# mrlooi/PoseCNN

Hardware: AMD Instinct MI355X
Metric: frames/sec 640x480x21-class Hough-vote+RoI+ADD-loss, 1/2/4/8 MI355X (higher is better)
Workload: dtype f32 (FC GEMMs: exact 3-way split-bf16 x6 MFMA, products within 2^-24, fp32 accumulate: fp32-faithful)

## Files before the change

include/posecnn_hip.h:

```cpp
#ifndef POSECNN_HIP_H
#define POSECNN_HIP_H

#include <stddef.h>
#include <stdint.h>

#ifdef __cplusplus
extern "C" {
#endif

#define PCNN_OK 0
#define PCNN_EINVAL 1
#define PCNN_EHIP 2
#define PCNN_ECAPACITY 3

#define PCNN_MAX_ROI 128

int pcnn_abi_version(void);
const char* pcnn_strerror(int code);

int pcnn_set_completion_event(void* event);
int pcnn_completion_event_pending(void);

size_t pcnn_hough_voting_workspace_size(int B, int H, int W, int C, int skip_pixels, float vote_thr);

// ... 35 lines not shown
int pcnn_roi_pool_fwd_pair(const float* data_a, int Ha, int Wa, float scale_a, const float* data_b, int Hb, int Wb,
                           float scale_b, int B, int C, const float* rois, int R_cap, int roi_stride,
                           int batch_base, const int32_t* num_rois_dev, int pooled_h, int pooled_w, float* top_sum,
                           int32_t* argmax_a, int32_t* argmax_b, void* stream);

int pcnn_roi_pool_fwd_pair_px(const float* data_a, int Ha, int Wa, float scale_a, const float* data_b, int Hb,
                              int Wb, float scale_b, int B, int C, const float* rois, int R_cap, int roi_stride,
                              int batch_base, const int32_t* num_rois_dev, int pooled_h, int pooled_w,
                              float* top_sum, uint16_t* argmax_a, uint16_t* argmax_b, void* stream);

size_t pcnn_roi_pool_bwd_workspace_size(int B, int R_cap);

int pcnn_roi_pool_bwd(const float* top_diff, const int32_t* argmax, int B, int H, int W, int C, int layout,
                      const float* rois, int R_cap, int roi_stride, int batch_base, const int32_t* num_rois_dev,
                      float spatial_scale, int pooled_h, int pooled_w, int pool_channel, float* bottom_diff,
                      void* workspace, size_t workspace_bytes, void* stream);

int pcnn_roi_pool_bwd_px(const float* top_diff, const uint16_t* argmax_px, int B, int H, int W, int C,
                         const float* rois, int R_cap, int roi_stride, int batch_base, const int32_t* num_rois_dev,
                         float spatial_scale, int pooled_h, int pooled_w, float* bottom_diff, void* workspace,
                         size_t workspace_bytes, void* stream);

size_t pcnn_add_loss_workspace_size(int R_cap, int C, int P);

int pcnn_add_loss_fwd(const float* pred, const float* target, const float* weight, const float* points,
                      const float* symmetry, int R_cap, const int32_t* num_rois_dev, int C, int P, float margin,
                      int loss_norm_rows, const int32_t* loss_norm_rows_dev, float* loss, float* bottom_diff,
                      void* workspace, size_t workspace_bytes, void* stream);

int pcnn_add_loss_prep(const float* weight, const float* symmetry, int R_cap, const int32_t* num_rois_dev, int C,
                       int P, void* workspace, size_t workspace_bytes, void* stream);
int pcnn_add_loss_fwd_prepared(const float* pred, const float* target, const float* weight, const float* points,
                               const float* symmetry, int R_cap, const int32_t* num_rois_dev, int C, int P,
                               float margin, int loss_norm_rows, const int32_t* loss_norm_rows_dev, float* loss,
                               float* bottom_diff, void* workspace, size_t workspace_bytes, void* stream);

int pcnn_add_loss_fwd_head_bwd(const float* pred, const float* target, const float* weight, const float* points,
                               const float* symmetry, int R_cap, const int32_t* num_rois_dev, int C, int P,
                               float margin, int loss_norm_rows, const int32_t* loss_norm_rows_dev,
                               float* bottom_diff, void* workspace, size_t workspace_bytes, const float* tanh_out,
                               const float* d_pred_scale, float* d_y8, void* stream);
int pcnn_add_loss_total(int R_cap, const int32_t* num_rois_dev, int C, int P, const void* workspace,
                        size_t workspace_bytes, float* loss, void* stream);

int pcnn_add_loss_bwd(const float* top_diff, const float* bottom_diff, int n, const int32_t* num_rois_dev,
                      int row_len, float* out, void* stream);
// ... 145 lines not shown
```

posecnn_amd/_lib.py:

```python
import ctypes
import os
import threading

import torch

_HERE = os.path.dirname(os.path.abspath(__file__))
LIB_PATH = os.environ.get("POSECNN_HIP_LIB") or os.path.join(_HERE, "libposecnn_hip.so")

_lib = None
_lock = threading.Lock()

c_int = ctypes.c_int
c_float = ctypes.c_float
c_size_t = ctypes.c_size_t
c_void_p = ctypes.c_void_p

_SIGS = {
    "pcnn_abi_version": (c_int, []),
    "pcnn_strerror": (ctypes.c_char_p, [c_int]),
    "pcnn_set_completion_event": (c_int, [c_void_p]),
    "pcnn_completion_event_pending": (c_int, []),
    "pcnn_hough_voting_workspace_size": (c_size_t, [c_int, c_int, c_int, c_int, c_int, c_float]),
    "pcnn_hough_voting": (c_int, [c_void_p, c_void_p, c_void_p, c_void_p, c_int, c_void_p, c_int, c_int, c_int,
                                  c_int, c_int, c_int, c_int, c_int, c_float, c_int, c_float, c_float, c_int,
# ... 5 lines not shown
                                       c_int, c_void_p, c_void_p, c_size_t, c_void_p]),
    "pcnn_hough_voting_compact": (c_int, [c_void_p, c_void_p, c_void_p, c_void_p, c_int, c_void_p, c_int, c_int,
                                          c_int, c_int, c_int, c_int, c_int, c_int, c_float, c_int, c_float, c_float,
                                          c_int, c_void_p, c_void_p, c_void_p, c_void_p, c_void_p, c_void_p, c_int,
                                          c_void_p, c_void_p, c_size_t, c_void_p]),
    "pcnn_hough_voting_grad": (c_int, [c_void_p, c_void_p, c_int, c_int, c_int, c_int, c_void_p]),
    "pcnn_hough_voting_diag": (c_int, [c_void_p, c_int, c_int, c_int, c_int, c_int, c_float, c_void_p, c_void_p]),
    "pcnn_roi_pool_fwd": (c_int, [c_void_p, c_int, c_int, c_int, c_int, c_int, c_void_p, c_int, c_int, c_int,
                                  c_void_p, c_float, c_int, c_int, c_int, c_void_p, c_void_p, c_void_p]),
    "pcnn_roi_pool_fwd_accumulate": (c_int, [c_void_p, c_int, c_int, c_int, c_int, c_int, c_void_p, c_int, c_int,
                                             c_int, c_void_p, c_float, c_int, c_int, c_int, c_void_p, c_void_p, c_void_p]),
    "pcnn_roi_pool_fwd_pair": (c_int, [c_void_p, c_int, c_int, c_float, c_void_p, c_int, c_int, c_float, c_int, c_int,
                                       c_void_p, c_int, c_int, c_int, c_void_p, c_int, c_int, c_void_p, c_void_p,
                                       c_void_p, c_void_p]),
    "pcnn_roi_pool_fwd_pair_px": (c_int, [c_void_p, c_int, c_int, c_float, c_void_p, c_int, c_int, c_float, c_int,
                                          c_int, c_void_p, c_int, c_int, c_int, c_void_p, c_int, c_int, c_void_p,
                                          c_void_p, c_void_p, c_void_p]),
    "pcnn_roi_pool_bwd_workspace_size": (c_size_t, [c_int, c_int]),
    "pcnn_roi_pool_bwd_px": (c_int, [c_void_p, c_void_p, c_int, c_int, c_int, c_int, c_void_p, c_int, c_int, c_int,
                                     c_void_p, c_float, c_int, c_int, c_void_p, c_void_p, c_size_t, c_void_p]),
    "pcnn_roi_pool_bwd": (c_int, [c_void_p, c_void_p, c_int, c_int, c_int, c_int, c_int, c_void_p, c_int, c_int,
                                  c_int, c_void_p, c_float, c_int, c_int, c_int, c_void_p, c_void_p, c_size_t, c_void_p]),
    "pcnn_add_loss_workspace_size": (c_size_t, [c_int, c_int, c_int]),
    "pcnn_add_loss_fwd": (c_int, [c_void_p, c_void_p, c_void_p, c_void_p, c_void_p, c_int, c_void_p, c_int, c_int,
                                  c_float, c_int, c_void_p, c_void_p, c_void_p, c_void_p, c_size_t, c_void_p]),
    "pcnn_add_loss_fwd_prepared": (c_int, [c_void_p, c_void_p, c_void_p, c_void_p, c_void_p, c_int, c_void_p, c_int, c_int,
                                  c_float, c_int, c_void_p, c_void_p, c_void_p, c_void_p, c_size_t, c_void_p]),
    "pcnn_add_loss_prep": (c_int, [c_void_p, c_void_p, c_int, c_void_p, c_int, c_int, c_void_p, c_size_t, c_void_p]),
    "pcnn_add_loss_fwd_head_bwd": (c_int, [c_void_p, c_void_p, c_void_p, c_void_p, c_void_p, c_int, c_void_p, c_int,
                                           c_int, c_float, c_int, c_void_p, c_void_p, c_void_p, c_size_t, c_void_p,
                                           c_void_p, c_void_p, c_void_p]),
    "pcnn_add_loss_total": (c_int, [c_int, c_void_p, c_int, c_int, c_void_p, c_size_t, c_void_p, c_void_p]),
    "pcnn_add_loss_bwd": (c_int, [c_void_p, c_void_p, c_int, c_void_p, c_int, c_void_p, c_void_p]),
    "pcnn_div_rn_check": (c_int, [c_void_p, c_float, c_int, c_int, c_void_p, c_void_p]),
    "pcnn_backproject_fwd": (c_int, [c_void_p, c_void_p, c_void_p, c_void_p, c_int, c_void_p, c_int, c_int, c_int,
                                     c_int, c_int, c_int, c_int, c_float, c_void_p, c_void_p, c_void_p, c_void_p]),
    "pcnn_backproject_bwd": (c_int, [c_void_p, c_void_p, c_void_p, c_int, c_int, c_int, c_int, c_int, c_int,
                                     c_void_p, c_void_p]),
    "pcnn_gemm_workspace_size": (c_size_t, [c_int, c_int, c_int, c_int, c_int]),
    "pcnn_gemm": (c_int, [c_int, c_int, c_int, c_void_p, c_void_p, c_int, c_int, c_void_p, c_int, c_int, c_void_p,
                          c_int, c_void_p, c_int, c_void_p, c_int, c_void_p, c_void_p, c_int, c_void_p, c_size_t,
                          c_void_p]),
    "pcnn_gemm_drop": (c_int, [c_int, c_int, c_int, c_void_p, c_void_p, c_int, c_int, c_void_p, c_int, c_int,
                               c_void_p, c_int, c_void_p, c_int, c_void_p, c_int, c_void_p, c_int, c_float, c_void_p,
                               c_void_p, c_int, c_void_p, c_size_t, c_void_p]),
    "pcnn_gemm_drop_gen": (c_int, [c_int, c_int, c_int, c_void_p, c_void_p, c_int, c_int, c_void_p, c_int, c_int,
# ... 141 lines not shown
```

posecnn_amd/average_distance_loss/average_distance_loss_op.py:

```python
import warnings

import torch

from .. import _lib


def workspace_bytes(R, num_classes, num_points):
    return _lib.load().pcnn_add_loss_workspace_size(R, num_classes, num_points)


def average_distance_loss_prep(bottom_weight, bottom_symmetry, num_points, workspace, num_rois=None, points=None):
    if points is not None:
        warnings.warn("average_distance_loss_prep: `points` is ignored (the pruned ADD-S search is removed)",
                      DeprecationWarning, stacklevel=2)
    _lib.require_gpu(bottom_weight, bottom_symmetry, workspace)
    w = bottom_weight.contiguous().float()
    R, PC = w.shape
    rc = _lib.load().pcnn_add_loss_prep(_lib.ptr(w), _lib.ptr(bottom_symmetry.contiguous().float()), R,
                                        _lib.ptr(num_rois), PC // 4, int(num_points), _lib.ptr(workspace),
                                        workspace.numel(), _lib.stream_ptr())
    _lib.check(rc, "average_distance_loss_prep")


def average_distance_loss(bottom_prediction, bottom_target, bottom_weight, bottom_point, bottom_symmetry, margin,
                          name=None, num_rois=None, loss_norm_rows=0, loss_norm_rows_dev=None, out=None,
                          workspace=None, prepared=False):
    _lib.require_gpu(bottom_prediction, bottom_target, bottom_weight, bottom_point, bottom_symmetry)
    if margin < 0:
        raise ValueError(f"Need margin >= 0, got {margin}")
    pred = bottom_prediction.contiguous().float()
    R, PC = pred.shape
# ... 64 lines not shown
```

posecnn_amd/csrc/average_distance.hip:

```cpp
#include "pcnn_common.h"
#include "head_common.h"
#include <cfloat>
#include <type_traits>

namespace {

#ifndef ADD_LANES
#define ADD_LANES 64
#endif
constexpr int kSymLanes = ADD_LANES;
#ifndef ADD_GRID
#define ADD_GRID 1024
#endif
#ifndef ADD_PPL
#define ADD_PPL 4
#endif
constexpr int kPPL = ADD_PPL;
constexpr int kPts = kSymLanes * kPPL;
constexpr int kMaxPointsLds = 8192;

__device__ __forceinline__ int rows_of(const int32_t* dev, int cap) {
  if (!dev) return cap;
  int r = *dev;
  return r < cap ? r : cap;
}
// ... 50 lines not shown
                                                float bn, float rbn, double ln, double rln, float* acc) {
  const float dist = (x1 - x2) * (x1 - x2) + (y1 - y2) * (y1 - y2) + (z1 - z2) * (z1 - z2);
  if (dist < margin) return;
  acc[0] += (float)div_rn((double)(dist - margin), ln, rln);
  const float d0[9] = {2 * s, -2 * w, 2 * v, 2 * w, 2 * s, -2 * u, -2 * v, 2 * u, 2 * s};
  const float d1[9] = {2 * u, 2 * v, 2 * w, 2 * v, -2 * u, -2 * s, 2 * w, 2 * s, -2 * u};
  const float d2[9] = {-2 * v, 2 * u, 2 * s, 2 * u, 2 * v, 2 * w, -2 * s, 2 * w, -2 * v};
  const float d3[9] = {-2 * w, -2 * s, 2 * u, 2 * s, -2 * w, 2 * v, 2 * u, 2 * v, 2 * w};
  const float X[3] = {X0, X1, X2};
  const float df[3] = {x1 - x2, y1 - y2, z1 - z2};
  float e0 = 0.f, e1 = 0.f, e2 = 0.f, e3 = 0.f;
#pragma unroll
  for (int a = 0; a < 3; a++)
#pragma unroll
    for (int b = 0; b < 3; b++) {
      e0 += div_rn(df[a] * X[b] * d0[a * 3 + b], bn, rbn);
      e1 += div_rn(df[a] * X[b] * d1[a * 3 + b], bn, rbn);
      e2 += div_rn(df[a] * X[b] * d2[a * 3 + b], bn, rbn);
      e3 += div_rn(df[a] * X[b] * d3[a * 3 + b], bn, rbn);
    }
  acc[1] += e0; acc[2] += e1; acc[3] += e2; acc[4] += e3;
}

__device__ __forceinline__ void add_plain_row(int n, const float* __restrict__ pred, const float* __restrict__ target,
                                              const float* __restrict__ points, const float* __restrict__ symmetry,
                                              int R, int C, int P, float margin, int norm_rows,
                                              const int32_t* __restrict__ norm_rows_dev, int nchunk,
                                              const int32_t* __restrict__ rcls, float* __restrict__ partial,
                                              float (*red)[5]) {
  const int cls = rcls[n];
  if (cls >= 0 && symmetry[cls] > 0) return;
  float* out = partial + (size_t)n * nchunk * 5;
  for (int i = threadIdx.x; i < nchunk * 5; i += blockDim.x) out[i] = 0.f;
  if (cls < 0) return;
  const int PC = 4 * C;
  const float* tq = target + (size_t)n * PC + 4 * cls;
  const float* pq = pred + (size_t)n * PC + 4 * cls;
  float Rg[9], Rp[9];
  quat2rot(tq[0], tq[1], tq[2], tq[3], Rg);
  const float s = pq[0], u = pq[1], v = pq[2], w = pq[3];
  quat2rot(s, u, v, w, Rp);
  const int Rn = norm_rows_dev ? *norm_rows_dev : (norm_rows > 0 ? norm_rows : R);
  const float bn = (float)(Rn * P), rbn = 1.f / bn;
  const double ln = 2.0 * (double)Rn * (double)P, rln = 1.0 / ln;
  const float* pts = points + (size_t)cls * P * 3;
  float acc[5] = {0.f, 0.f, 0.f, 0.f, 0.f};
  for (int p = threadIdx.x; p < P; p += blockDim.x) {
    const float X0 = pts[p * 3 + 0], X1 = pts[p * 3 + 1], X2 = pts[p * 3 + 2];
    const float x1 = Rp[0] * X0 + Rp[1] * X1 + Rp[2] * X2;
    const float y1 = Rp[3] * X0 + Rp[4] * X1 + Rp[5] * X2;
    const float z1 = Rp[6] * X0 + Rp[7] * X1 + Rp[8] * X2;
    const float x2 = Rg[0] * X0 + Rg[1] * X1 + Rg[2] * X2;
    const float y2 = Rg[3] * X0 + Rg[4] * X1 + Rg[5] * X2;
    const float z2 = Rg[6] * X0 + Rg[7] * X1 + Rg[8] * X2;
    add_point_terms(X0, X1, X2, x1, y1, z1, x2, y2, z2, s, u, v, w, margin, bn, rbn, ln, rln, acc);
  }
#pragma unroll
  for (int q = 0; q < 5; q++) acc[q] = pcnn::wave_sum(acc[q]);
  if (pcnn::lane_id() == 0)
    for (int q = 0; q < 5; q++) red[threadIdx.x >> 6][q] = acc[q];
  __syncthreads();
  if (threadIdx.x < 5) {
    float t = 0.f;
    for (int i = 0; i < (int)(blockDim.x >> 6); i++) t += red[i][threadIdx.x];
    out[threadIdx.x] = t;
  }
}

#ifndef ADD_GROUPS
#define ADD_GROUPS 4
#endif
constexpr int kSymGroups = ADD_GROUPS;
constexpr int kSymThreads = kSymLanes * kSymGroups;
#ifndef ADD_BLK
#define ADD_BLK 8
#endif
constexpr int kBlk = ADD_BLK;

__global__ void __launch_bounds__(kSymThreads) k_add_rows(const float* __restrict__ pred,
                                                           const float* __restrict__ target,
                                                           const float* __restrict__ weight,
                                                           const float* __restrict__ points,
                                                           const float* __restrict__ symmetry, int R_cap,
                                                           const int32_t* __restrict__ num_rois_dev, int C, int P,
                                                           float margin, int norm_rows,
                                                           const int32_t* __restrict__ norm_rows_dev, int nchunk,
                                                           const int32_t* __restrict__ rcls,
                                                           const int32_t* __restrict__ sym_rows,
                                                           const int32_t* __restrict__ nsym,
                                                           int32_t* __restrict__ queue,
                                                           float* __restrict__ partial) {
  extern __shared__ __attribute__((aligned(16))) float4 gpts[];
  __shared__ float mdist[kSymGroups - 1][kPts];
  __shared__ int midx[kSymGroups - 1][kPts];
  __shared__ float red[kSymThreads / 64][5];
  __shared__ int s_imin[kPts];
  const int R = rows_of(num_rois_dev, R_cap);
  const int sym_items = *nsym * nchunk;
  const int items = sym_items + R;
  const int grp = threadIdx.x / kSymLanes, lt = threadIdx.x % kSymLanes;
  const int quarter = ((P + kSymGroups - 1) / kSymGroups + kBlk - 1) / kBlk * kBlk;
  const int c0 = grp * quarter, c1 = min(P, c0 + quarter);
  __shared__ int s_item;
  for (;;) {
  __syncthreads();
  if (threadIdx.x == 0) s_item = atomicAdd(queue, 1);
  __syncthreads();
  const int item = s_item;
  if (item >= items) break;
  if (item >= sym_items) {
    add_plain_row(item - sym_items, pred, target, points, symmetry, R, C, P, margin, norm_rows, norm_rows_dev,
                  nchunk, rcls, partial, red);
    continue;
  }
  const int nfull = P / kPts, nsym_rows = *nsym;
  int n, chunk, slot;
  if (item < nsym_rows * nfull) {
    slot = item / nfull;
    chunk = item % nfull;
  } else {
    slot = item - nsym_rows * nfull;
    chunk = nfull;
  }
  n = sym_rows[slot];
  const int PC = 4 * C;
  const int cls = rcls[n];
  float* out = partial + ((size_t)n * nchunk + chunk) * 5;
  const float* tq = target + (size_t)n * PC + 4 * cls;
  const float* pq = pred + (size_t)n * PC + 4 * cls;
  float Rg[9], Rp[9];
  quat2rot(tq[0], tq[1], tq[2], tq[3], Rg);
  const float s = pq[0], u = pq[1], v = pq[2], w = pq[3];
  quat2rot(s, u, v, w, Rp);
  const float* pts = points + (size_t)cls * P * 3;
  for (int i = threadIdx.x; i < P; i += blockDim.x) {
    const float X0 = pts[i * 3 + 0], X1 = pts[i * 3 + 1], X2 = pts[i * 3 + 2];
    gpts[i] = make_float4(Rg[0] * X0 + Rg[1] * X1 + Rg[2] * X2, Rg[3] * X0 + Rg[4] * X1 + Rg[5] * X2,
                          Rg[6] * X0 + Rg[7] * X1 + Rg[8] * X2, 0.f);
  }
  __syncthreads();
  float qx[kPPL], qy[kPPL], qz[kPPL], Xq[kPPL][3];
  int pq_[kPPL];
#pragma unroll
  for (int k = 0; k < kPPL; k++) {
    const int p = chunk * kPts + k * kSymLanes + lt;
    pq_[k] = p;
    const int pp = p < P ? p : 0;
    Xq[k][0] = pts[pp * 3 + 0]; Xq[k][1] = pts[pp * 3 + 1]; Xq[k][2] = pts[pp * 3 + 2];
    qx[k] = Rp[0] * Xq[k][0] + Rp[1] * Xq[k][1] + Rp[2] * Xq[k][2];
    qy[k] = Rp[3] * Xq[k][0] + Rp[4] * Xq[k][1] + Rp[5] * Xq[k][2];
    qz[k] = Rp[6] * Xq[k][0] + Rp[7] * Xq[k][1] + Rp[8] * Xq[k][2];
  }
  auto dist_to = [&](int k, const float4& c) {
    return (qx[k] - c.x) * (qx[k] - c.x) + (qy[k] - c.y) * (qy[k] - c.y) + (qz[k] - c.z) * (qz[k] - c.z);
  };
  float dmin[kPPL];
  int iblk[kPPL];
#pragma unroll
  for (int k = 0; k < kPPL; k++) { dmin[k] = FLT_MAX; iblk[k] = -1; }
  typedef float f2 __attribute__((ext_vector_type(2)));
  f2 px[kPPL / 2], py[kPPL / 2], pz[kPPL / 2];
#pragma unroll
  for (int h = 0; h < kPPL / 2; h++) {
// ... 15 lines not shown
        for (int j = 0; j < kBlk; j++) {
          const f2 ex = px[h] - c[j].x, ey = py[h] - c[j].y, ez = pz[h] - c[j].z;
          d[j] = ex * ex + ey * ey + ez * ez;
        }
#pragma unroll
        for (int e = 0; e < 2; e++) {
          const int k = 2 * h + e;
          float bm = fminf(d[0][e], d[1][e]);
#pragma unroll
          for (int j = 2; j < kBlk; j += 2) bm = fminf(bm, fminf(d[j][e], d[j + 1][e]));
          if (bm < dmin[k]) { dmin[k] = bm; iblk[k] = i; }
        }
      }
    }
    for (; i < c1; i++) {
      const float4 c = gpts[i];
#pragma unroll
      for (int k = 0; k < 2 * NP; k++) {
        const float d = dist_to(k, c);
        if (d < dmin[k]) { dmin[k] = d; iblk[k] = i; }
      }
    }
  };
  const int nq = min(kPts, P - chunk * kPts);
  if (nq > 2 * kSymLanes) scan(std::integral_constant<int, kPPL / 2>{});
  else scan(std::integral_constant<int, 1>{});
  if (grp > 0) {
#pragma unroll
    for (int k = 0; k < kPPL; k++) {
      mdist[grp - 1][k * kSymLanes + lt] = dmin[k];
      midx[grp - 1][k * kSymLanes + lt] = iblk[k];
    }
  }
  __syncthreads();
  if (grp == 0) {
#pragma unroll
    for (int k = 0; k < kPPL; k++) {
#pragma unroll
      for (int g = 0; g < kSymGroups - 1; g++) {
        const float d = mdist[g][k * kSymLanes + lt];
        if (d < dmin[k]) { dmin[k] = d; iblk[k] = midx[g][k * kSymLanes + lt]; }
      }
      int im = -1;
      if (iblk[k] >= 0) {
        const int e = min(iblk[k] + kBlk, P);
        for (int j = iblk[k]; j < e; j++)
          if (dist_to(k, gpts[j]) == dmin[k]) { im = j; break; }
      }
      s_imin[k * kSymLanes + lt] = im;
    }
  }
  __syncthreads();
  float acc[5] = {0.f, 0.f, 0.f, 0.f, 0.f};
  for (int jj = threadIdx.x; jj < kPts; jj += blockDim.x) {
    const int p = chunk * kPts + jj;
    if (p >= P) continue;
    const int im = s_imin[jj] < 0 ? p : s_imin[jj];
    const float X0 = pts[p * 3 + 0], X1 = pts[p * 3 + 1], X2 = pts[p * 3 + 2];
    const float x1 = Rp[0] * X0 + Rp[1] * X1 + Rp[2] * X2;
    const float y1 = Rp[3] * X0 + Rp[4] * X1 + Rp[5] * X2;
    const float z1 = Rp[6] * X0 + Rp[7] * X1 + Rp[8] * X2;
    const float4 cm = gpts[im];
    const int Rn = norm_rows_dev ? *norm_rows_dev : (norm_rows > 0 ? norm_rows : R);
    const float bn = (float)(Rn * P), rbn = 1.f / bn;
    const double ln = 2.0 * (double)Rn * (double)P, rln = 1.0 / ln;
    add_point_terms(X0, X1, X2, x1, y1, z1, cm.x, cm.y, cm.z, s, u, v, w, margin, bn, rbn, ln, rln, acc);
  }
#pragma unroll
  for (int q = 0; q < 5; q++) acc[q] = pcnn::wave_sum(acc[q]);
  if (pcnn::lane_id() == 0)
    for (int q = 0; q < 5; q++) red[threadIdx.x >> 6][q] = acc[q];
  __syncthreads();
  if (threadIdx.x < 5) {
    float t = 0.f;
    for (int i = 0; i < kSymThreads / 64; i++) t += red[i][threadIdx.x];
    out[threadIdx.x] = t;
  }
  __syncthreads();
  }
}

__global__ void __launch_bounds__(1024) k_add_prep(const float* __restrict__ weight, const float* __restrict__ symmetry,
                                                    int R_cap, const int32_t* __restrict__ num_rois_dev, int C,
                                                    int32_t* __restrict__ rcls, int32_t* __restrict__ sym_rows,
                                                    int32_t* __restrict__ nsym, int32_t* __restrict__ queue) {
  __shared__ int wcount[16];
  __shared__ int base;
  const int R = rows_of(num_rois_dev, R_cap);
  const int lane = pcnn::lane_id(), wave = threadIdx.x >> 6;
  if (threadIdx.x == 0) base = 0;
  __syncthreads();
  for (int n0 = 0; n0 < R; n0 += blockDim.x) {
    const int n = n0 + threadIdx.x;
    int cls = -1;
    if (n < R) {
      cls = row_class(weight, n, C);
      rcls[n] = cls;
    }
    const bool sym = n < R && cls >= 0 && symmetry[cls] > 0;
    const uint64_t m = __ballot(sym);
    if (lane == 0) wcount[wave] = __popcll(m);
    __syncthreads();
    int off = base;
    for (int w = 0; w < wave; w++) off += wcount[w];
    if (sym) sym_rows[off + __popcll(m & pcnn::lanemask_lt())] = n;
    __syncthreads();
    if (threadIdx.x == 0) {
      int t = 0;
      for (int w = 0; w < (int)(blockDim.x >> 6); w++) t += wcount[w];
      base += t;
    }
    __syncthreads();
  }
  if (threadIdx.x == 0) {
    *nsym = base;
    *queue = 0;
  }
}

__device__ __forceinline__ void fold_row(int n, int nchunk, const float* __restrict__ partial, int lane, float* s) {
#pragma unroll
  for (int q = 0; q < 5; q++) s[q] = 0.f;
  for (int k = lane; k < nchunk; k += 64)
    for (int q = 0; q < 5; q++) s[q] += partial[((size_t)n * nchunk + k) * 5 + q];
#pragma unroll
  for (int q = 0; q < 5; q++) s[q] = pcnn::wave_sum(s[q]);
}

__device__ __forceinline__ void finish_row(int n, int R, int C, int nchunk, const int32_t* __restrict__ rcls,
                                           const float* __restrict__ partial, float* __restrict__ row_loss,
                                           float* __restrict__ bottom_diff, int lane) {
  if (n >= R) return;
  const int cls = rcls[n];
  float s[5];
  fold_row(n, nchunk, partial, lane, s);
  const int PC = 4 * C;
  for (int col = lane; col < PC; col += 64) {
    float vv = 0.f;
    if (cls >= 0 && col >= 4 * cls && col < 4 * cls + 4) vv = s[1 + col - 4 * cls];
// ... 67 lines not shown

__global__ void k_add_bwd_rows(const float* __restrict__ top_diff, const float* __restrict__ bottom_diff,
                               const int32_t* __restrict__ num_rois_dev, int R_cap, int row_len,
                               float* __restrict__ out) {
  const float g = top_diff[0];
  const int n = rows_of(num_rois_dev, R_cap) * row_len;
  for (int i = blockIdx.x * blockDim.x + threadIdx.x; i < n; i += gridDim.x * blockDim.x) out[i] = g * bottom_diff[i];
}

}

extern "C" int pcnn_div_rn_check(const float* x, float b, int n, int dbl, float* out, void* stream) {
  PCNN_REQUIRE(x && out && n >= 0 && b != 0.f);
  if (n == 0) return PCNN_OK;
  hipLaunchKernelGGL(k_div_rn_check, dim3((n + 255) / 256), dim3(256), 0, (hipStream_t)stream, x, b, n, dbl, out);
  PCNN_CHECK_LAUNCH();
  return PCNN_OK;
}

struct AddWs {
  float* partial;
  int32_t *rcls, *sym_rows, *nsym, *queue;
  float* row_loss;
};
static AddWs add_carve(void* workspace, int R_cap, int P, size_t* bytes) {
  const int nchunk = (P + kPts - 1) / kPts;
  const size_t R = (size_t)(R_cap > 0 ? R_cap : 1);
  pcnn::Carve cv(workspace);
  AddWs w;
  w.partial = cv.take<float>(R * nchunk * 5);
  w.rcls = cv.take<int32_t>(R);
  w.sym_rows = cv.take<int32_t>(R);
  w.nsym = cv.take<int32_t>(1);
  w.queue = cv.take<int32_t>(1);
  w.row_loss = cv.take<float>(R);
  if (bytes) *bytes = cv.off + 256;
  return w;
}

extern "C" size_t pcnn_add_loss_workspace_size(int R_cap, int C, int P) {
  (void)C;
  size_t b = 0;
  (void)add_carve(nullptr, R_cap, P, &b);
  return b;
}

static void add_launch_prep(const AddWs& w, const float* weight, const float* symmetry, int R_cap,
                            const int32_t* num_rois_dev, int C, hipStream_t st) {
  hipLaunchKernelGGL(k_add_prep, dim3(1), dim3(1024), 0, st, weight, symmetry, R_cap, num_rois_dev, C, w.rcls,
                     w.sym_rows, w.nsym, w.queue);
}

static void add_launch_rows(const AddWs& w, const float* pred, const float* target, const float* weight,
                            const float* points, const float* symmetry, int R_cap, const int32_t* num_rois_dev,
                            int C, int P, float margin, int loss_norm_rows, const int32_t* loss_norm_rows_dev,
                            hipStream_t st) {
  const int nchunk = (P + kPts - 1) / kPts;
  const long items = (long)R_cap * nchunk + R_cap;
  const int grid = (int)(items < ADD_GRID ? items : ADD_GRID);
  hipLaunchKernelGGL(k_add_rows, dim3(grid), dim3(kSymThreads), (size_t)P * sizeof(float4), st, pred, target,
                     weight, points, symmetry, R_cap, num_rois_dev, C, P, margin, loss_norm_rows,
                     loss_norm_rows_dev, nchunk, w.rcls, w.sym_rows, w.nsym, w.queue, w.partial);
}

static int add_loss_fwd(const float* pred, const float* target, const float* weight, const float* points,
                        const float* symmetry, int R_cap, const int32_t* num_rois_dev, int C, int P, float margin,
                        int loss_norm_rows, const int32_t* loss_norm_rows_dev, float* loss, float* bottom_diff,
                        void* workspace, size_t workspace_bytes, bool prepared, void* stream) {
  PCNN_REQUIRE(pred && target && weight && points && symmetry && loss && bottom_diff && workspace);
  PCNN_REQUIRE(R_cap > 0 && C > 0 && P > 0 && P <= kMaxPointsLds);
  if (workspace_bytes < pcnn_add_loss_workspace_size(R_cap, C, P)) return PCNN_ECAPACITY;
  hipStream_t st = (hipStream_t)stream;
  const int nchunk = (P + kPts - 1) / kPts;
  const AddWs w = add_carve(workspace, R_cap, P, nullptr);
  if (!prepared) add_launch_prep(w, weight, symmetry, R_cap, num_rois_dev, C, st);
  add_launch_rows(w, pred, target, weight, points, symmetry, R_cap, num_rois_dev, C, P, margin, loss_norm_rows,
                  loss_norm_rows_dev, st);
  hipLaunchKernelGGL(k_add_finish_rows, dim3((R_cap + 3) / 4), dim3(256), 0, st, R_cap, num_rois_dev, C, nchunk,
                     w.rcls, w.partial, w.row_loss, bottom_diff);
  hipLaunchKernelGGL(k_add_total, dim3(1), dim3(1024), 0, st, R_cap, num_rois_dev, w.row_loss, loss);
  PCNN_CHECK_LAUNCH();
  return PCNN_OK;
}

extern "C" int pcnn_add_loss_fwd(const float* pred, const float* target, const float* weight, const float* points,
                                 const float* symmetry, int R_cap, const int32_t* num_rois_dev, int C, int P,
                                 float margin, int loss_norm_rows, const int32_t* loss_norm_rows_dev, float* loss,
                                 float* bottom_diff, void* workspace, size_t workspace_bytes, void* stream) {
  return add_loss_fwd(pred, target, weight, points, symmetry, R_cap, num_rois_dev, C, P, margin, loss_norm_rows,
                      loss_norm_rows_dev, loss, bottom_diff, workspace, workspace_bytes, false, stream);
}

extern "C" int pcnn_add_loss_prep(const float* weight, const float* symmetry, int R_cap, const int32_t* num_rois_dev,
                                  int C, int P, void* workspace, size_t workspace_bytes, void* stream) {
  PCNN_REQUIRE(weight && symmetry && workspace && R_cap > 0 && C > 0 && P > 0 && P <= kMaxPointsLds);
  if (workspace_bytes < pcnn_add_loss_workspace_size(R_cap, C, P)) return PCNN_ECAPACITY;
  const AddWs w = add_carve(workspace, R_cap, P, nullptr);
  add_launch_prep(w, weight, symmetry, R_cap, num_rois_dev, C, (hipStream_t)stream);
  PCNN_CHECK_LAUNCH();
  return PCNN_OK;
}

extern "C" int pcnn_add_loss_fwd_prepared(const float* pred, const float* target, const float* weight,
                                          const float* points, const float* symmetry, int R_cap,
                                          const int32_t* num_rois_dev, int C, int P, float margin,
                                          int loss_norm_rows, const int32_t* loss_norm_rows_dev, float* loss,
                                          float* bottom_diff, void* workspace, size_t workspace_bytes,
// ... 53 lines not shown
```

Before: 4485.

## Use MFMA-based candidate filtering for symmetric ADD-loss nearest-point search

Replaces the brute-force nearest-neighbour scan for symmetric classes with a two-stage search. A split-bf16 MFMA pass computes approximate distances per 32-point block, keeps only blocks within a window of the per-query minimum, and then evaluates those candidates exactly in fp32 with atomicMin on packed distance-index keys. The kernel is templated on the filter path with larger blocks and more LDS, falls back to the scan when inputs are out of range or LDS is insufficient, and packs two plain rows per block. It also adds search statistics counters, at the cost of more code complexity and a dependency on the bf16 window bound holding for exactness.

```diff
diff --git a/include/posecnn_hip.h b/include/posecnn_hip.h
--- a/include/posecnn_hip.h
+++ b/include/posecnn_hip.h
@@ -81,6 +81,7 @@
                          size_t workspace_bytes, void* stream);
 
 size_t pcnn_add_loss_workspace_size(int R_cap, int C, int P);
+size_t pcnn_add_loss_stats_offset(int R_cap, int C, int P);
 
 int pcnn_add_loss_fwd(const float* pred, const float* target, const float* weight, const float* points,
                       const float* symmetry, int R_cap, const int32_t* num_rois_dev, int C, int P, float margin,
diff --git a/posecnn_amd/_lib.py b/posecnn_amd/_lib.py
--- a/posecnn_amd/_lib.py
+++ b/posecnn_amd/_lib.py
@@ -51,6 +51,7 @@
     "pcnn_roi_pool_bwd": (c_int, [c_void_p, c_void_p, c_int, c_int, c_int, c_int, c_int, c_void_p, c_int, c_int,
                                   c_int, c_void_p, c_float, c_int, c_int, c_int, c_void_p, c_void_p, c_size_t, c_void_p]),
     "pcnn_add_loss_workspace_size": (c_size_t, [c_int, c_int, c_int]),
+    "pcnn_add_loss_stats_offset": (c_size_t, [c_int, c_int, c_int]),
     "pcnn_add_loss_fwd": (c_int, [c_void_p, c_void_p, c_void_p, c_void_p, c_void_p, c_int, c_void_p, c_int, c_int,
                                   c_float, c_int, c_void_p, c_void_p, c_void_p, c_void_p, c_size_t, c_void_p]),
     "pcnn_add_loss_fwd_prepared": (c_int, [c_void_p, c_void_p, c_void_p, c_void_p, c_void_p, c_int, c_void_p, c_int, c_int,
diff --git a/posecnn_amd/average_distance_loss/average_distance_loss_op.py b/posecnn_amd/average_distance_loss/average_distance_loss_op.py
--- a/posecnn_amd/average_distance_loss/average_distance_loss_op.py
+++ b/posecnn_amd/average_distance_loss/average_distance_loss_op.py
@@ -7,6 +7,12 @@
 
 def workspace_bytes(R, num_classes, num_points):
     return _lib.load().pcnn_add_loss_workspace_size(R, num_classes, num_points)
+
+
+def search_stats(workspace, R, num_classes, num_points):
+    off = _lib.load().pcnn_add_loss_stats_offset(R, num_classes, num_points)
+    f, s, t = workspace[off:off + 12].cpu().view(torch.int32).tolist()
+    return {"filter_items": f, "scan_items": s, "triples": t, "exact_evals": 16 * t}
 
 
 def average_distance_loss_prep(bottom_weight, bottom_symmetry, num_points, workspace, num_rois=None, points=None):
diff --git a/posecnn_amd/csrc/average_distance.hip b/posecnn_amd/csrc/average_distance.hip
--- a/posecnn_amd/csrc/average_distance.hip
+++ b/posecnn_amd/csrc/average_distance.hip
@@ -1,6 +1,9 @@
 #include "pcnn_common.h"
 #include "head_common.h"
+#include <atomic>
 #include <cfloat>
+#include <cstdlib>
+#include <cstring>
 #include <type_traits>
 
 namespace {
@@ -97,48 +100,55 @@
   acc[1] += e0; acc[2] += e1; acc[3] += e2; acc[4] += e3;
 }
 
-__device__ __forceinline__ void add_plain_row(int n, const float* __restrict__ pred, const float* __restrict__ target,
-                                              const float* __restrict__ points, const float* __restrict__ symmetry,
-                                              int R, int C, int P, float margin, int norm_rows,
-                                              const int32_t* __restrict__ norm_rows_dev, int nchunk,
-                                              const int32_t* __restrict__ rcls, float* __restrict__ partial,
-                                              float (*red)[5]) {
-  const int cls = rcls[n];
-  if (cls >= 0 && symmetry[cls] > 0) return;
-  float* out = partial + (size_t)n * nchunk * 5;
-  for (int i = threadIdx.x; i < nchunk * 5; i += blockDim.x) out[i] = 0.f;
-  if (cls < 0) return;
-  const int PC = 4 * C;
-  const float* tq = target + (size_t)n * PC + 4 * cls;
-  const float* pq = pred + (size_t)n * PC + 4 * cls;
-  float Rg[9], Rp[9];
-  quat2rot(tq[0], tq[1], tq[2], tq[3], Rg);
-  const float s = pq[0], u = pq[1], v = pq[2], w = pq[3];
-  quat2rot(s, u, v, w, Rp);
-  const int Rn = norm_rows_dev ? *norm_rows_dev : (norm_rows > 0 ? norm_rows : R);
-  const float bn = (float)(Rn * P), rbn = 1.f / bn;
-  const double ln = 2.0 * (double)Rn * (double)P, rln = 1.0 / ln;
-  const float* pts = points + (size_t)cls * P * 3;
+template <int kRows>
+__device__ __forceinline__ void add_plain_rows(int n0, const float* __restrict__ pred,
+                                               const float* __restrict__ target, const float* __restrict__ points,
+                                               const float* __restrict__ symmetry, int R, int C, int P, float margin,
+                                               int norm_rows, const int32_t* __restrict__ norm_rows_dev, int nchunk,
+                                               const int32_t* __restrict__ rcls, float* __restrict__ partial,
+                                               float (*red)[5]) {
+  const int half = kRows == 2 ? (int)(threadIdx.x / kPts) : 0, tid = (int)(threadIdx.x % kPts);
+  const int n = n0 + half;
+  const bool live = n < R;
+  const int cls = live ? rcls[n] : -1;
+  const bool sym = cls >= 0 && symmetry[cls] > 0;
+  float* out = partial + (size_t)(live ? n : 0) * nchunk * 5;
+  if (live && !sym)
+    for (int i = tid; i < nchunk * 5; i += kPts) out[i] = 0.f;
+  const bool work = live && !sym && cls >= 0;
   float acc[5] = {0.f, 0.f, 0.f, 0.f, 0.f};
-  for (int p = threadIdx.x; p < P; p += blockDim.x) {
-    const float X0 = pts[p * 3 + 0], X1 = pts[p * 3 + 1], X2 = pts[p * 3 + 2];
-    const float x1 = Rp[0] * X0 + Rp[1] * X1 + Rp[2] * X2;
-    const float y1 = Rp[3] * X0 + Rp[4] * X1 + Rp[5] * X2;
-    const float z1 = Rp[6] * X0 + Rp[7] * X1 + Rp[8] * X2;
-    const float x2 = Rg[0] * X0 + Rg[1] * X1 + Rg[2] * X2;
-    const float y2 = Rg[3] * X0 + Rg[4] * X1 + Rg[5] * X2;
-    const float z2 = Rg[6] * X0 + Rg[7] * X1 + Rg[8] * X2;
-    add_point_terms(X0, X1, X2, x1, y1, z1, x2, y2, z2, s, u, v, w, margin, bn, rbn, ln, rln, acc);
+  if (work) {
+    const int PC = 4 * C;
+    const float* tq = target + (size_t)n * PC + 4 * cls;
+    const float* pq = pred + (size_t)n * PC + 4 * cls;
+    float Rg[9], Rp[9];
+    quat2rot(tq[0], tq[1], tq[2], tq[3], Rg);
+    const float s = pq[0], u = pq[1], v = pq[2], w = pq[3];
+    quat2rot(s, u, v, w, Rp);
+    const int Rn = norm_rows_dev ? *norm_rows_dev : (norm_rows > 0 ? norm_rows : R);
+    const float bn = (float)(Rn * P), rbn = 1.f / bn;
+    const double ln = 2.0 * (double)Rn * (double)P, rln = 1.0 / ln;
+    const float* pts = points + (size_t)cls * P * 3;
+    for (int p = tid; p < P; p += kPts) {
+      const float X0 = pts[p * 3 + 0], X1 = pts[p * 3 + 1], X2 = pts[p * 3 + 2];
+      const float x1 = Rp[0] * X0 + Rp[1] * X1 + Rp[2] * X2;
+      const float y1 = Rp[3] * X0 + Rp[4] * X1 + Rp[5] * X2;
+      const float z1 = Rp[6] * X0 + Rp[7] * X1 + Rp[8] * X2;
+      const float x2 = Rg[0] * X0 + Rg[1] * X1 + Rg[2] * X2;
+      const float y2 = Rg[3] * X0 + Rg[4] * X1 + Rg[5] * X2;
+      const float z2 = Rg[6] * X0 + Rg[7] * X1 + Rg[8] * X2;
+      add_point_terms(X0, X1, X2, x1, y1, z1, x2, y2, z2, s, u, v, w, margin, bn, rbn, ln, rln, acc);
+    }
   }
 #pragma unroll
   for (int q = 0; q < 5; q++) acc[q] = pcnn::wave_sum(acc[q]);
   if (pcnn::lane_id() == 0)
     for (int q = 0; q < 5; q++) red[threadIdx.x >> 6][q] = acc[q];
   __syncthreads();
-  if (threadIdx.x < 5) {
+  if (work && tid < 5) {
     float t = 0.f;
-    for (int i = 0; i < (int)(blockDim.x >> 6); i++) t += red[i][threadIdx.x];
-    out[threadIdx.x] = t;
+    for (int i = 0; i < kPts / 64; i++) t += red[half * (kPts / 64) + i][tid];
+    out[tid] = t;
   }
 }
 
@@ -152,7 +162,191 @@
 #endif
 constexpr int kBlk = ADD_BLK;
 
-__global__ void __launch_bounds__(kSymThreads) k_add_rows(const float* __restrict__ pred,
+typedef unsigned u32x4 __attribute__((ext_vector_type(4)));
+typedef float f32x16 __attribute__((ext_vector_type(16)));
+typedef __bf16 bf16x8 __attribute__((ext_vector_type(8)));
+
+constexpr int kFiltWaves = 8;
+constexpr int kFiltThreads = 64 * kFiltWaves;
+constexpr int kFiltMaxPoints = 2816;
+constexpr int kFiltList = 1024;
+constexpr int kFiltBlk = ((kFiltMaxPoints + 31) / 32 + kFiltWaves - 1) / kFiltWaves;
+constexpr float kFiltWin = 2.8e-4f;
+constexpr float kFiltM2Min = 0x1p-40f, kFiltM2Max = 0x1p40f;
+constexpr unsigned kFiltPadNorm = 0x7180u;
+
+template <bool F>
+struct FiltLds {};
+template <>
+struct FiltLds<true> {
+  float4 sq[kPts];
+  float smin[kFiltWaves][kPts];
+  unsigned long long skey[kPts];
+  unsigned list[kFiltList];
+  int cnt, m2;
+};
+
+__device__ __forceinline__ unsigned bf16_rn(float x) {
+  const unsigned b = __float_as_uint(x);
+  return (b + 0x7fffu + ((b >> 16) & 1u)) >> 16;
+}
+__device__ __forceinline__ float bf16_val(unsigned h) { return __uint_as_float(h << 16); }
+__device__ __forceinline__ void bf16_split2(float x, unsigned& h, unsigned& m) {
+  h = bf16_rn(x);
+  m = bf16_rn(x - bf16_val(h));
+}
+
+__device__ __forceinline__ void filt_candidate(const float4& c, float n, u32x4& k0, u32x4& k8) {
+  unsigned xh, xm, yh, ym, zh, zm;
+  bf16_split2(c.x, xh, xm);
+  bf16_split2(c.y, yh, ym);
+  bf16_split2(c.z, zh, zm);
+  const unsigned nh = bf16_rn(n);
+  const float r1 = n - bf16_val(nh);
+  const unsigned nm = bf16_rn(r1);
+  const unsigned nl = bf16_rn(r1 - bf16_val(nm));
+  k0 = (u32x4){xh | xh << 16, xm | xm << 16, yh | yh << 16, ym | ym << 16};
+  k8 = (u32x4){zh | zh << 16, zm | zm << 16, nh | nm << 16, nl};
+}
+
+__device__ __forceinline__ float filt_min17(float m, const f32x16& v) {
+  float a = fminf(fminf(v[0], v[1]), v[2]);
+  float b = fminf(fminf(v[3], v[4]), v[5]);
+  a = fminf(fminf(a, v[6]), v[7]);
+  b = fminf(fminf(b, v[8]), v[9]);
+  a = fminf(fminf(a, v[10]), v[11]);
+  b = fminf(fminf(b, v[12]), v[13]);
+  a = fminf(fminf(a, v[14]), v[15]);
+  return fminf(fminf(m, a), b);
+}
+
+template <int NF>
+__device__ __forceinline__ int filter_search(FiltLds<true>& fl, const float4* gpts, const char* cimg, int P, int nq,
+                                             float win, int* s_imin) {
+  const int lane = pcnn::lane_id(), r = lane & 31, h = lane >> 5;
+  const int wave = __builtin_amdgcn_readfirstlane((int)(threadIdx.x >> 6));
+  const int nblk = (P + 31) >> 5, bq = nblk / kFiltWaves, brem = nblk % kFiltWaves;
+  const int b0 = wave * bq + min(wave, brem), b1 = b0 + bq + (wave < brem ? 1 : 0);
+  bf16x8 qb[NF];
+#pragma unroll
+  for (int f = 0; f < NF; f++) {
+    const float4 q = fl.sq[f * 32 + r];
+    unsigned xh, xm, yh, ym, zh, zm;
+    bf16_split2(-2.f * q.x, xh, xm);
+    bf16_split2(-2.f * q.y, yh, ym);
+    bf16_split2(-2.f * q.z, zh, zm);
+    const u32x4 w = h == 0 ? (u32x4){xh | xm << 16, xh | xm << 16, yh | ym << 16, yh | ym << 16}
+                           : (u32x4){zh | zm << 16, zh | zm << 16, 0x3f803f80u, 0x00003f80u};
+    qb[f] = __builtin_bit_cast(bf16x8, w);
+  }
+  const f32x16 zero = {0.f, 0.f, 0.f, 0.f, 0.f, 0.f, 0.f, 0.f, 0.f, 0.f, 0.f, 0.f, 0.f, 0.f, 0.f, 0.f};
+  const char* ap = cimg + r * 32 + h * 16;
+  float bmin[kFiltBlk][NF];
+  bf16x8 a = *(const bf16x8*)(ap + min(b0, nblk - 1) * 1024);
+#pragma unroll
+  for (int k = 0; k < kFiltBlk; k++) {
+    if (b0 + k < b1) {
+      const bf16x8 an = *(const bf16x8*)(ap + min(b0 + k + 1, nblk - 1) * 1024);
+      f32x16 v = __builtin_amdgcn_mfma_f32_32x32x16_bf16(a, qb[0], zero, 0, 0, 0);
+#pragma unroll
+      for (int f = 0; f < NF; f++) {
+        f32x16 vn = v;
+        if (f + 1 < NF) vn = __builtin_amdgcn_mfma_f32_32x32x16_bf16(a, qb[f + 1], zero, 0, 0, 0);
+        __builtin_amdgcn_sched_barrier(0);
+        bmin[k][f] = filt_min17(FLT_MAX, v);
+        __builtin_amdgcn_sched_barrier(0);
+        v = vn;
+      }
+      a = an;
+    } else {
+#pragma unroll
+      for (int f = 0; f < NF; f++) bmin[k][f] = FLT_MAX;
+    }
+  }
+#pragma unroll
+  for (int f = 0; f < NF; f++) {
+    float m = bmin[0][f];
+#pragma unroll
+    for (int k = 1; k < kFiltBlk; k++) m = fminf(m, bmin[k][f]);
+    m = fminf(m, __shfl_xor(m, 32, 64));
+    if (h == 0) fl.smin[wave][f * 32 + r] = m;
+  }
+  __syncthreads();
+  unsigned mask[NF];
+#pragma unroll
+  for (int f = 0; f < NF; f++) {
+    float t = fl.smin[0][f * 32 + r];
+#pragma unroll
+    for (int g = 1; g < kFiltWaves; g++) t = fminf(t, fl.smin[g][f * 32 + r]);
+    const float thr = t + win;
+    unsigned mk = 0u;
+#pragma unroll
+    for (int k = 0; k < kFiltBlk; k++) mk |= bmin[k][f] <= thr ? 1u << k : 0u;
+    mask[f] = mk;
+  }
+#pragma unroll
+  for (int f = 0; f < NF; f++)
+    if (f * 32 + r >= nq) mask[f] = 0u;
+  int nrec = 0;
+  for (;;) {
+    int mine = 0;
+#pragma unroll
+    for (int f = 0; f < NF; f++) mine += __popc(mask[f]);
+    int incl = mine;
+#pragma unroll
+    for (int o = 1; o < 64; o <<= 1) {
+      const int t = __shfl_up(incl, o, 64);
+      if (lane >= o) incl += t;
+    }
+    const int total = __shfl(incl, 63, 64);
+    int base = 0;
+    if (lane == 0 && total > 0) base = atomicAdd(&fl.cnt, total);
+    int pos = __shfl(base, 0, 64) + incl - mine;
+    int pending = 0;
+#pragma unroll
+    for (int f = 0; f < NF; f++) {
+      unsigned mk = mask[f];
+      while (mk && pos < kFiltList) {
+        const int bit = __ffs(mk) - 1;
+        mk &= mk - 1;
+        fl.list[pos++] = (unsigned)(f * 32 + r) << 16 | (unsigned)(b0 + bit) << 1 | (unsigned)h;
+      }
+      mask[f] = mk;
+      pending |= mk != 0u;
+    }
+    __syncthreads();
+    const int n = min(fl.cnt, kFiltList);
+    for (int w = threadIdx.x; w < n; w += blockDim.x) {
+      const unsigned rec = fl.list[w];
+      const int qi = rec >> 16;
+      const int i0 = (int)((rec >> 1) & 0x7fffu) * 32 + 4 * (int)(rec & 1u);
+      const float4 q = fl.sq[qi];
+      unsigned long long best = ~0ull;
+#pragma unroll
+      for (int reg = 0; reg < 16; reg++) {
+        const int idx = i0 + (reg & 3) + 8 * (reg >> 2);
+        const float4 c = gpts[min(idx, P - 1)];
+        const float d = (q.x - c.x) * (q.x - c.x) + (q.y - c.y) * (q.y - c.y) + (q.z - c.z) * (q.z - c.z);
+        const unsigned long long key = (unsigned long long)__float_as_uint(d) << 32 | (unsigned long long)(unsigned)idx;
+        if (idx < P && d < FLT_MAX && key < best) best = key;
+      }
+      if (best != ~0ull) atomicMin(&fl.skey[qi], best);
+    }
+    nrec += n;
+    pending = __syncthreads_or(pending);
+    if (!pending) break;
+    if (threadIdx.x == 0) fl.cnt = 0;
+    __syncthreads();
+  }
+  if (threadIdx.x < kPts) {
+    const unsigned long long key = fl.skey[threadIdx.x];
+    s_imin[threadIdx.x] = key == ~0ull ? -1 : (int)(unsigned)(key & 0xffffffffull);
+  }
+  return nrec;
+}
+
+template <bool kFilt>
+__global__ void __launch_bounds__(kFilt ? kFiltThreads : kSymThreads) k_add_rows(const float* __restrict__ pred,
                                                            const float* __restrict__ target,
                                                            const float* __restrict__ weight,
                                                            const float* __restrict__ points,
@@ -164,28 +358,35 @@
                                                            const int32_t* __restrict__ sym_rows,
                                                            const int32_t* __restrict__ nsym,
                                                            int32_t* __restrict__ queue,
+                                                           int32_t* __restrict__ stats,
                                                            float* __restrict__ partial) {
   extern __shared__ __attribute__((aligned(16))) float4 gpts[];
+  __shared__ FiltLds<kFilt> fl;
   __shared__ float mdist[kSymGroups - 1][kPts];
   __shared__ int midx[kSymGroups - 1][kPts];
-  __shared__ float red[kSymThreads / 64][5];
+  __shared__ float red[(kFilt ? kFiltThreads : kSymThreads) / 64][5];
   __shared__ int s_imin[kPts];
   const int R = rows_of(num_rois_dev, R_cap);
   const int sym_items = *nsym * nchunk;
-  const int items = sym_items + R;
+  constexpr int kPlain = kFilt ? kFiltThreads / kPts : 1;
+  const int items = sym_items + (R + kPlain - 1) / kPlain;
   const int grp = threadIdx.x / kSymLanes, lt = threadIdx.x % kSymLanes;
   const int quarter = ((P + kSymGroups - 1) / kSymGroups + kBlk - 1) / kBlk * kBlk;
   const int c0 = grp * quarter, c1 = min(P, c0 + quarter);
   __shared__ int s_item;
+  int st_filter = 0, st_scan = 0, st_triples = 0;
   for (;;) {
   __syncthreads();
-  if (threadIdx.x == 0) s_item = atomicAdd(queue, 1);
+  if (threadIdx.x == 0) {
+    s_item = atomicAdd(queue, 1);
+    if constexpr (kFilt) { fl.cnt = 0; fl.m2 = 0; }
+  }
   __syncthreads();
   const int item = s_item;
   if (item >= items) break;
   if (item >= sym_items) {
-    add_plain_row(item - sym_items, pred, target, points, symmetry, R, C, P, margin, norm_rows, norm_rows_dev,
-                  nchunk, rcls, partial, red);
+    add_plain_rows<kPlain>((item - sym_items) * kPlain, pred, target, points, symmetry, R, C, P, margin, norm_rows,
+                           norm_rows_dev, nchunk, rcls, partial, red);
     continue;
   }
   const int nfull = P / kPts, nsym_rows = *nsym;
@@ -208,12 +409,72 @@
   const float s = pq[0], u = pq[1], v = pq[2], w = pq[3];
   quat2rot(s, u, v, w, Rp);
   const float* pts = points + (size_t)cls * P * 3;
+  const int nq = min(kPts, P - chunk * kPts);
+  bool searched = false;
+  int nrec = 0;
+  float Xt0 = 0.f, Xt1 = 0.f, Xt2 = 0.f;
+  if constexpr (kFilt) {
+    char* cimg = (char*)gpts + (((size_t)P * sizeof(float4) + 31) & ~(size_t)31);
+    const int Ppad = (P + 31) & ~31;
+    float mx = 0.f;
+    int bad = 0;
+    constexpr int kStage = (kFiltMaxPoints + kFiltThreads - 1) / kFiltThreads;
+    float Xs[kStage][3];
+#pragma unroll
+    for (int k = 0; k < kStage; k++) {
+      const int i = (int)threadIdx.x + k * kFiltThreads;
+      const int ii = i < P ? i : 0;
+      Xs[k][0] = pts[ii * 3 + 0]; Xs[k][1] = pts[ii * 3 + 1]; Xs[k][2] = pts[ii * 3 + 2];
+    }
+#pragma unroll
+    for (int k = 0; k < kStage; k++) {
+      const int i = (int)threadIdx.x + k * kFiltThreads;
+      if (i >= Ppad) continue;
+      u32x4 k0 = {0u, 0u, 0u, 0u}, k8 = {0u, 0u, kFiltPadNorm, 0u};
+      if (i < P) {
+        const float X0 = Xs[k][0], X1 = Xs[k][1], X2 = Xs[k][2];
+        const float4 c = make_float4(Rg[0] * X0 + Rg[1] * X1 + Rg[2] * X2, Rg[3] * X0 + Rg[4] * X1 + Rg[5] * X2,
+                                     Rg[6] * X0 + Rg[7] * X1 + Rg[8] * X2, 0.f);
+        gpts[i] = c;
+        const float nn = c.x * c.x + c.y * c.y + c.z * c.z;
+        bad |= !(nn <= kFiltM2Max);
+        mx = fmaxf(mx, nn);
+        filt_candidate(c, nn, k0, k8);
+      }
+      *(u32x4*)(cimg + (size_t)i * 32) = k0;
+      *(u32x4*)(cimg + (size_t)i * 32 + 16) = k8;
+    }
+    if (threadIdx.x < kPts) {
+      const int p = chunk * kPts + (int)threadIdx.x;
+      const int pp = p < P ? p : 0;
+      const float X0 = pts[pp * 3 + 0], X1 = pts[pp * 3 + 1], X2 = pts[pp * 3 + 2];
+      Xt0 = X0; Xt1 = X1; Xt2 = X2;
+      const float4 q = make_float4(Rp[0] * X0 + Rp[1] * X1 + Rp[2] * X2, Rp[3] * X0 + Rp[4] * X1 + Rp[5] * X2,
+                                   Rp[6] * X0 + Rp[7] * X1 + Rp[8] * X2, 0.f);
+      fl.sq[threadIdx.x] = q;
+      const float nn = q.x * q.x + q.y * q.y + q.z * q.z;
+      bad |= !(nn <= kFiltM2Max);
+      mx = fmaxf(mx, nn);
+      fl.skey[threadIdx.x] = ~0ull;
+    }
+    mx = pcnn::wave_max(mx);
+    if (pcnn::lane_id() == 0) atomicMax(&fl.m2, __float_as_int(mx));
+    bad = __syncthreads_or(bad);
+    const float m2 = __int_as_float(fl.m2);
+    if (!bad && m2 >= kFiltM2Min) {
+      nrec = nq > 64 ? filter_search<8>(fl, gpts, cimg, P, nq, kFiltWin * m2, s_imin)
+                     : filter_search<2>(fl, gpts, cimg, P, nq, kFiltWin * m2, s_imin);
+      searched = true;
+    }
+  } else {
   for (int i = threadIdx.x; i < P; i += blockDim.x) {
     const float X0 = pts[i * 3 + 0], X1 = pts[i * 3 + 1], X2 = pts[i * 3 + 2];
     gpts[i] = make_float4(Rg[0] * X0 + Rg[1] * X1 + Rg[2] * X2, Rg[3] * X0 + Rg[4] * X1 + Rg[5] * X2,
                           Rg[6] * X0 + Rg[7] * X1 + Rg[8] * X2, 0.f);
   }
   __syncthreads();
+  }
+  if (!searched) {
   float qx[kPPL], qy[kPPL], qz[kPPL], Xq[kPPL][3];
   int pq_[kPPL];
 #pragma unroll
@@ -275,10 +536,9 @@
       }
     }
   };
-  const int nq = min(kPts, P - chunk * kPts);
   if (nq > 2 * kSymLanes) scan(std::integral_constant<int, kPPL / 2>{});
   else scan(std::integral_constant<int, 1>{});
-  if (grp > 0) {
+  if (grp > 0 && grp < kSymGroups) {
 #pragma unroll
     for (int k = 0; k < kPPL; k++) {
       mdist[grp - 1][k * kSymLanes + lt] = dmin[k];
@@ -303,13 +563,15 @@
       s_imin[k * kSymLanes + lt] = im;
     }
   }
+  }
   __syncthreads();
   float acc[5] = {0.f, 0.f, 0.f, 0.f, 0.f};
   for (int jj = threadIdx.x; jj < kPts; jj += blockDim.x) {
     const int p = chunk * kPts + jj;
     if (p >= P) continue;
     const int im = s_imin[jj] < 0 ? p : s_imin[jj];
-    const float X0 = pts[p * 3 + 0], X1 = pts[p * 3 + 1], X2 = pts[p * 3 + 2];
+    static_assert(kPts == kSymThreads, "one tail point per thread: jj == threadIdx.x");
+    const float X0 = kFilt ? Xt0 : pts[p * 3 + 0], X1 = kFilt ? Xt1 : pts[p * 3 + 1], X2 = kFilt ? Xt2 : pts[p * 3 + 2];
     const float x1 = Rp[0] * X0 + Rp[1] * X1 + Rp[2] * X2;
     const float y1 = Rp[3] * X0 + Rp[4] * X1 + Rp[5] * X2;
     const float z1 = Rp[6] * X0 + Rp[7] * X1 + Rp[8] * X2;
@@ -321,7 +583,7 @@
   }
 #pragma unroll
   for (int q = 0; q < 5; q++) acc[q] = pcnn::wave_sum(acc[q]);
-  if (pcnn::lane_id() == 0)
+  if (pcnn::lane_id() == 0 && threadIdx.x < kSymThreads)
     for (int q = 0; q < 5; q++) red[threadIdx.x >> 6][q] = acc[q];
   __syncthreads();
   if (threadIdx.x < 5) {
@@ -329,14 +591,26 @@
     for (int i = 0; i < kSymThreads / 64; i++) t += red[i][threadIdx.x];
     out[threadIdx.x] = t;
   }
-  __syncthreads();
+  if (searched) {
+    st_filter++;
+    st_triples += nrec;
+  } else {
+    st_scan++;
+  }
+  __syncthreads();
+  }
+  if (threadIdx.x == 0) {
+    if (st_filter) atomicAdd(stats + 0, st_filter);
+    if (st_scan) atomicAdd(stats + 1, st_scan);
+    if (st_triples) atomicAdd(stats + 2, st_triples);
   }
 }
 
 __global__ void __launch_bounds__(1024) k_add_prep(const float* __restrict__ weight, const float* __restrict__ symmetry,
                                                     int R_cap, const int32_t* __restrict__ num_rois_dev, int C,
                                                     int32_t* __restrict__ rcls, int32_t* __restrict__ sym_rows,
-                                                    int32_t* __restrict__ nsym, int32_t* __restrict__ queue) {
+                                                    int32_t* __restrict__ nsym, int32_t* __restrict__ queue,
+                                                    int32_t* __restrict__ stats) {
   __shared__ int wcount[16];
   __shared__ int base;
   const int R = rows_of(num_rois_dev, R_cap);
@@ -368,6 +642,7 @@
   if (threadIdx.x == 0) {
     *nsym = base;
     *queue = 0;
+    stats[0] = stats[1] = stats[2] = 0;
   }
 }
 
@@ -481,6 +756,8 @@
   float* partial;
   int32_t *rcls, *sym_rows, *nsym, *queue;
   float* row_loss;
+  int32_t* stats;
+  size_t stats_off;
 };
 static AddWs add_carve(void* workspace, int R_cap, int P, size_t* bytes) {
   const int nchunk = (P + kPts - 1) / kPts;
@@ -493,6 +770,8 @@
   w.nsym = cv.take<int32_t>(1);
   w.queue = cv.take<int32_t>(1);
   w.row_loss = cv.take<float>(R);
+  w.stats = cv.take<int32_t>(4);
+  w.stats_off = cv.off - 4 * sizeof(int32_t);
   if (bytes) *bytes = cv.off + 256;
   return w;
 }
@@ -507,7 +786,37 @@
 static void add_launch_prep(const AddWs& w, const float* weight, const float* symmetry, int R_cap,
                             const int32_t* num_rois_dev, int C, hipStream_t st) {
   hipLaunchKernelGGL(k_add_prep, dim3(1), dim3(1024), 0, st, weight, symmetry, R_cap, num_rois_dev, C, w.rcls,
-                     w.sym_rows, w.nsym, w.queue);
+                     w.sym_rows, w.nsym, w.queue, w.stats);
+}
+
+static size_t add_filter_lds(int P) {
+  return (((size_t)P * sizeof(float4) + 31) & ~(size_t)31) + (size_t)((P + 31) & ~31) * 32;
+}
+
+static bool add_use_filter(int P) {
+  const char* mode = getenv("PCNN_ADD_SEARCH");
+  if (mode && strcmp(mode, "scan") == 0) return false;
+  if (P > kFiltMaxPoints) return false;
+  static std::atomic<int> room[pcnn::kMaxDevices];
+  int dev = 0;
+  if (hipGetDevice(&dev) != hipSuccess || dev < 0 || dev >= pcnn::kMaxDevices) return false;
+  int have = room[dev].load(std::memory_order_acquire);
+  if (have == 0) {
+    hipFuncAttributes fa;
+    int lds = 0;
+    have = -1;
+    if (hipFuncGetAttributes(&fa, (const void*)k_add_rows<true>) == hipSuccess &&
+        hipDeviceGetAttribute(&lds, hipDeviceAttributeMaxSharedMemoryPerBlock, dev) == hipSuccess &&
+        lds > (int)fa.sharedSizeBytes) {
+      const int dyn = lds - (int)fa.sharedSizeBytes;
+      if (hipFuncSetAttribute((const void*)k_add_rows<true>, hipFuncAttributeMaxDynamicSharedMemorySize, dyn) ==
+          hipSuccess)
+        have = dyn;
+    }
+    if (have < 0) (void)hipGetLastError();
+    room[dev].store(have, std::memory_order_release);
+  }
+  return have > 0 && add_filter_lds(P) <= (size_t)have;
 }
 
 static void add_launch_rows(const AddWs& w, const float* pred, const float* target, const float* weight,
@@ -517,9 +826,14 @@
   const int nchunk = (P + kPts - 1) / kPts;
   const long items = (long)R_cap * nchunk + R_cap;
   const int grid = (int)(items < ADD_GRID ? items : ADD_GRID);
-  hipLaunchKernelGGL(k_add_rows, dim3(grid), dim3(kSymThreads), (size_t)P * sizeof(float4), st, pred, target,
-                     weight, points, symmetry, R_cap, num_rois_dev, C, P, margin, loss_norm_rows,
-                     loss_norm_rows_dev, nchunk, w.rcls, w.sym_rows, w.nsym, w.queue, w.partial);
+  if (add_use_filter(P))
+    hipLaunchKernelGGL(k_add_rows<true>, dim3(grid), dim3(kFiltThreads), add_filter_lds(P), st, pred, target, weight,
+                       points, symmetry, R_cap, num_rois_dev, C, P, margin, loss_norm_rows, loss_norm_rows_dev,
+                       nchunk, w.rcls, w.sym_rows, w.nsym, w.queue, w.stats, w.partial);
+  else
+    hipLaunchKernelGGL(k_add_rows<false>, dim3(grid), dim3(kSymThreads), (size_t)P * sizeof(float4), st, pred,
+                       target, weight, points, symmetry, R_cap, num_rois_dev, C, P, margin, loss_norm_rows,
+                       loss_norm_rows_dev, nchunk, w.rcls, w.sym_rows, w.nsym, w.queue, w.stats, w.partial);
 }
 
 static int add_loss_fwd(const float* pred, const float* target, const float* weight, const float* points,
@@ -542,6 +856,11 @@
   return PCNN_OK;
 }
 
+extern "C" size_t pcnn_add_loss_stats_offset(int R_cap, int C, int P) {
+  (void)C;
+  return add_carve(nullptr, R_cap, P, nullptr).stats_off;
+}
+
 extern "C" int pcnn_add_loss_fwd(const float* pred, const float* target, const float* weight, const float* points,
                                  const float* symmetry, int R_cap, const int32_t* num_rois_dev, int C, int P,
                                  float margin, int loss_norm_rows, const int32_t* loss_norm_rows_dev, float* loss,
```

After: 4544, median of 6. 1.01x the previous value.
